# KVM-Explorer/AscendPathTracing

Hardware: AMD Instinct MI355X
Metric: Mray/s (ray segments per second) at 1920x1080, 8 bounces, 256 spp, demo scene (higher is better)
Workload: dtype f32; 1 GPU; C2: gen_spheres() 8-sphere scene, 1920x1080, S=64 (256 spp), depth 8, rays generated on device (counter RNG, seed 0), K-mode arithmetic, all segments traced (no retirement); segments_per_gpu=4246732800, parallelism=single GPU

## Files before the change

ascendpathtracing_amd/csrc/pt_trace2.h:

```cpp
#pragma once
#include <type_traits>

#include "pt_trace.h"

namespace {

template <bool PLANES, bool FIRST> constexpr int kPairSkip = !PLANES ? 0 : FIRST ? 0x8 : 0x80;
template <bool PLANES, bool FIRST> constexpr int kPairSkipLastB = 0;

struct PathPair {
    f2 ox, oy, oz, dx, dy, dz;
    f2 rx, ry, rz;
};

__device__ __forceinline__ PathState unpack_path(const PathPair &p, int which, uint64_t alive, bool first) {
    PathState s;
    if (which == 0) path_init(s, p.ox.x, p.oy.x, p.oz.x, p.dx.x, p.dy.x, p.dz.x);
    else path_init(s, p.ox.y, p.oy.y, p.oz.y, p.dx.y, p.dy.y, p.dz.y);
    if (first) return s;
    s.rxy = which == 0 ? f2{p.rx.x, p.ry.x} : f2{p.rx.y, p.ry.y};
    s.rz = which == 0 ? p.rz.x : p.rz.y;
    s.alive = select_const(alive, 1);
    return s;
}

template <int MODE, bool PLANES, bool FIRST>
__device__ __forceinline__ void bounce2_ns8_t(const Scene8 &sc, const Tab8 tab, const PathPair &s, PathPair &n,
                                              const TraceArgs &ta, const KeyConsts &kc, uint32_t ones_off,
                                              uint64_t &aliveA, uint64_t &aliveB, uint64_t &redoA, uint64_t &redoB) {
    float aminA = 1.0f, aminB = 1.0f;
    const Hit8 hA = intersect_ns8_v2<MODE, PLANES, kPairSkip<PLANES, FIRST>>(sc, s.ox.x, s.oy.x, s.oz.x, s.dx.x, s.dy.x, s.dz.x, ta, kc, aminA);
    const Hit8 hB = intersect_ns8_v2<MODE, PLANES, kPairSkip<PLANES, FIRST>>(sc, s.ox.y, s.oy.y, s.oz.y, s.dx.y, s.dy.y, s.dz.y, ta, kc, aminB);
    if (FIRST) {
        aliveA = ~hA.light;
        aliveB = ~hB.light;
    } else {
        aliveA &= ~hA.light;
        aliveB &= ~hB.light;
    }
    const char *geo = reinterpret_cast<const char *>(tab.geo);
    uint32_t cA, cB;
    asm("v_cndmask_b32_e64 %0, %1, %2, %3" : "=v"(cA) : "v"(ones_off), "v"(hA.addr), "s"(aliveA));
    asm("v_cndmask_b32_e64 %0, %1, %2, %3" : "=v"(cB) : "v"(ones_off), "v"(hB.addr), "s"(aliveB));
    const uint32_t gA = (uint32_t)(uintptr_t)geo + hA.addr, gB = (uint32_t)(uintptr_t)geo + hB.addr;
    const uint32_t aA = (uint32_t)(uintptr_t)geo + cA, aB = (uint32_t)(uintptr_t)geo + cB;
    float cxA, cyA, czA, cxB, cyB, czB, axA, ayA, azA, axB, ayB, azB;
    asm volatile("ds_read_b32 %0, %12\n ds_read_b32 %1, %12 offset:4\n ds_read_b32 %2, %12 offset:8\n"
                 "ds_read_b32 %3, %13\n ds_read_b32 %4, %13 offset:4\n ds_read_b32 %5, %13 offset:8\n"
                 "ds_read_b32 %6, %14 offset:128\n ds_read_b32 %7, %14 offset:132\n ds_read_b32 %8, %14 offset:136\n"
                 "ds_read_b32 %9, %15 offset:128\n ds_read_b32 %10, %15 offset:132\n ds_read_b32 %11, %15 offset:136\n"
                 "s_waitcnt lgkmcnt(0)"
                 : "=&v"(cxA), "=&v"(cyA), "=&v"(czA), "=&v"(cxB), "=&v"(cyB), "=&v"(czB), "=&v"(axA), "=&v"(ayA), "=&v"(azA),
                   "=&v"(axB), "=&v"(ayB), "=&v"(azB)
                 : "v"(gA), "v"(gB), "v"(aA), "v"(aB)
                 : "memory");
    const f2 cx = {cxA, cxB}, cy = {cyA, cyB}, cz = {czA, czB};
    const f2 ax = {axA, axB}, ay = {ayA, ayB}, az = {azA, azB};
    const f2 t = {hA.tmin, hB.tmin};
    const f2 hx = s.ox + s.dx * t, hy = s.oy + s.dy * t, hz = s.oz + s.dz * t;
    const f2 nx = hx - cx, ny = hy - cy, nz = hz - cz;
    f2 len2;
    if (MODE == kModeOracle) {
        const f2 p0 = nx * nx, p1 = ny * ny, p2 = nz * nz;
        len2 = f2{sum3_f64(p0.x, p1.x, p2.x), sum3_f64(p0.y, p1.y, p2.y)};
    } else {
        len2 = nx * nx + ny * ny;
        len2 = len2 + nz * nz;
    }
    const f2 r0 = {__builtin_amdgcn_rsqf(len2.x), __builtin_amdgcn_rsqf(len2.y)};
    aminA = minimum3_abs_after_trans(aminA, r0.x, nx.x);
    aminA = minimum3_abs(aminA, ny.x, nz.x);
    aminB = minimum3_abs_after_trans(aminB, r0.y, nx.y);
    aminB = minimum3_abs(aminB, ny.y, nz.y);
    const f2 L = sqrt_rsq_step(len2, r0);
    f2 ux, uy, uz, e1;
    div3_seeded_packed2(nx, ny, nz, L, r0, ux, uy, uz, e1);
    f2 dot;
    if (MODE == kModeOracle) {
        const f2 p0 = s.dx * ux, p1 = s.dy * uy, p2 = s.dz * uz;
        dot = f2{sum3_f64(p0.x, p1.x, p2.x), sum3_f64(p0.y, p1.y, p2.y)};
    } else {
        dot = s.dx * ux;
        dot = dot + s.dy * uy;
        dot = dot + s.dz * uz;
    }
    const f2 k2 = twice_canonical(dot);
    n.dx = s.dx - ux * k2; n.dy = s.dy - uy * k2; n.dz = s.dz - uz * k2;
    n.ox = hx; n.oy = hy; n.oz = hz;
    if (FIRST) { n.rx = ax; n.ry = ay; n.rz = az; }
    else { n.rx = ax * s.rx; n.ry = ay * s.ry; n.rz = az * s.rz; }
    redoA = __builtin_amdgcn_ballot_w64(!(aminA >= kFastMin)) | __builtin_amdgcn_ballot_w64(e1.x == kDiv3SeededStuck);
    redoB = __builtin_amdgcn_ballot_w64(!(aminB >= kFastMin)) | __builtin_amdgcn_ballot_w64(e1.y == kDiv3SeededStuck);
}
template <int MODE, bool PLANES>
__device__ __forceinline__ void bounce2_ns8(const Scene8 &sc, const Tab8 tab, const PathPair &s, PathPair &n,
                                            const TraceArgs &ta, const KeyConsts &kc, uint32_t ones_off,
                                            uint64_t &aliveA, uint64_t &aliveB, uint64_t &redoA, uint64_t &redoB) {
    bounce2_ns8_t<MODE, PLANES, false>(sc, tab, s, n, ta, kc, ones_off, aliveA, aliveB, redoA, redoB);
}
template <int MODE, bool PLANES>
__device__ __forceinline__ void bounce2_ns8_first(const Scene8 &sc, const Tab8 tab, const PathPair &s, PathPair &n,
                                                  const TraceArgs &ta, const KeyConsts &kc, uint32_t ones_off,
                                                  uint64_t &aliveA, uint64_t &aliveB, uint64_t &redoA, uint64_t &redoB) {
    bounce2_ns8_t<MODE, PLANES, true>(sc, tab, s, n, ta, kc, ones_off, aliveA, aliveB, redoA, redoB);
}

template <int MODE, bool PLANES, bool FIRST = false>
__device__ __forceinline__ void bounce2_ns8_last(const Scene8 &sc, const Tab8 tab, const PathPair &s, f2 &rx, f2 &ry, f2 &rz,
                                                 const TraceArgs &ta, const KeyConsts &kc, uint32_t ones_off,
                                                 uint64_t &aliveA, uint64_t &aliveB, uint64_t &redoA, uint64_t &redoB) {
    float aminA = 1.0f, aminB = 1.0f;
    const Hit8 hA = intersect_ns8_v2<MODE, PLANES, kPairSkip<PLANES, FIRST>>(sc, s.ox.x, s.oy.x, s.oz.x, s.dx.x, s.dy.x, s.dz.x, ta, kc, aminA);
    const Hit8 hB = intersect_ns8_v2<MODE, PLANES, kPairSkipLastB<PLANES, FIRST>>(sc, s.ox.y, s.oy.y, s.oz.y, s.dx.y, s.dy.y, s.dz.y, ta, kc, aminB);
    if (FIRST) {
        aliveA = ~hA.light;
        aliveB = ~hB.light;
    } else {
        aliveA &= ~hA.light;
        aliveB &= ~hB.light;
    }
    uint32_t cA, cB;
    asm("v_cndmask_b32_e64 %0, %1, %2, %3" : "=v"(cA) : "v"(ones_off), "v"(hA.addr), "s"(aliveA));
    asm("v_cndmask_b32_e64 %0, %1, %2, %3" : "=v"(cB) : "v"(ones_off), "v"(hB.addr), "s"(aliveB));
    const char *geo = reinterpret_cast<const char *>(tab.geo);
    const uint32_t aA = (uint32_t)(uintptr_t)geo + cA, aB = (uint32_t)(uintptr_t)geo + cB;
    float axA, ayA, azA, axB, ayB, azB;
    asm volatile("ds_read_b32 %0, %6 offset:128\n ds_read_b32 %1, %6 offset:132\n ds_read_b32 %2, %6 offset:136\n"
                 "ds_read_b32 %3, %7 offset:128\n ds_read_b32 %4, %7 offset:132\n ds_read_b32 %5, %7 offset:136\n"
                 "s_waitcnt lgkmcnt(0)"
                 : "=&v"(axA), "=&v"(ayA), "=&v"(azA), "=&v"(axB), "=&v"(ayB), "=&v"(azB)
                 : "v"(aA), "v"(aB)
                 : "memory");
    if (FIRST) { rx = f2{axA, axB}; ry = f2{ayA, ayB}; rz = f2{azA, azB}; }
    else { rx = f2{axA, axB} * s.rx; ry = f2{ayA, ayB} * s.ry; rz = f2{azA, azB} * s.rz; }
    redoA = __builtin_amdgcn_ballot_w64(!(aminA >= kFastMin));
    redoB = __builtin_amdgcn_ballot_w64(!(aminB >= kFastMin));
}

template <int MODE, bool PLANES>
__device__ __forceinline__ void trace2_ns8_t(const Scene8 &sc, const Tab8 tab, PathPair &s, const TraceArgs &ta) {
    const KeyConsts kc = make_key_consts(ta.eps);
    uint32_t ones_off = 8 * 16;
    asm volatile("" : "+v"(ones_off));
    uint64_t aliveA = __builtin_amdgcn_ballot_w64(true), aliveB = aliveA;
    const bool fast_ok = eps_allows_rootkey(ta.eps);
    auto redo_stands = [&](const PathPair &in, uint64_t redoA, uint64_t redoB, bool first) __attribute__((always_inline)) {
        if (first) return (redoA | redoB) != 0;
        const bool finA = select_const(aliveA, 1) == 0 || (in.rx.x == 0.0f && in.ry.x == 0.0f && in.rz.x == 0.0f);
        const bool finB = select_const(aliveB, 1) == 0 || (in.rx.y == 0.0f && in.ry.y == 0.0f && in.rz.y == 0.0f);
        return __builtin_amdgcn_ballot_w64((select_const(redoA, 1) != 0 && !finA) || (select_const(redoB, 1) != 0 && !finB)) != 0;
    };
    auto exact_pair = [&](const PathPair &in, PathState &na, PathState &nb, bool first) __attribute__((always_inline)) {
        PathState a = unpack_path(in, 0, aliveA, first), b = unpack_path(in, 1, aliveB, first);
        bounce_ns8_exact<MODE>(sc, tab, a, na, ta);
        bounce_ns8_exact<MODE>(sc, tab, b, nb, ta);
        if (ta.traced && (threadIdx.x & 63) == 0) atomicAdd(ta.traced + 3, 1ull);
    };
#ifdef APT_COUNT_PAIR_SKIP
    uint32_t count_bounce = 0;
    auto count_pairs = [&](const PathPair &in) __attribute__((always_inline)) {
        if (!ta.traced) return;
        const bool lane0 = (threadIdx.x & 63) == 0;
        for (int half = 0; half < 2; ++half) {
            const float ox = half ? in.ox.y : in.ox.x, oy = half ? in.oy.y : in.oy.x, oz = half ? in.oz.y : in.oz.x;
            const float dx = half ? in.dx.y : in.dx.x, dy = half ? in.dy.y : in.dy.x, dz = half ? in.dz.y : in.dz.x;
            HitPre2 hp[4];
            f2 c67 = {0.0f, 0.0f};
            if (PLANES) intersect_pre_planes<true>(sc, ox, oy, oz, dx, dy, dz, hp, &c67);
            for (int k = 0; k < 8; k += 2) {
                const HitPre2 h = PLANES ? hp[k / 2]
                                         : intersect_pre2(f2{sc.cx[k], sc.cx[k + 1]}, f2{sc.cy[k], sc.cy[k + 1]}, f2{sc.cz[k], sc.cz[k + 1]},
                                                          f2{sc.r2[k], sc.r2[k + 1]}, ox, oy, oz, dx, dy, dz);
                const uint32_t slot = 4u + (uint32_t)(half * 8 + (count_bounce < 7u ? count_bounce : 7u)) * 4u + (uint32_t)(k / 2);
                if (pair_misses_wave(h.disc) && lane0) atomicAdd(ta.traced + slot, 1ull);
                if (PLANES && k == 6) {
                    const uint32_t s67 = 72u + (uint32_t)(half * 8 + (count_bounce < 7u ? count_bounce : 7u)) * 4u;
                    const bool u6 = sphere_reachable_mask(h.disc.x, h.b.x, c67.x) == 0, u7 = sphere_reachable_mask(h.disc.y, h.b.y, c67.y) == 0;
                    const bool r6 = h.disc.x >= 0.0f && !(h.b.x < 0.0f && c67.x > 0.0f), r7 = h.disc.y >= 0.0f && !(h.b.y < 0.0f && c67.y > 0.0f);
                    const bool plain = __builtin_amdgcn_ballot_w64(r6 || r7) == 0;
                    if (u6 && lane0) atomicAdd(ta.traced + s67, 1ull);
                    if (u7 && lane0) atomicAdd(ta.traced + s67 + 1, 1ull);
                    if (u6 && u7 && lane0) atomicAdd(ta.traced + s67 + 2, 1ull);
                    if (plain && lane0) atomicAdd(ta.traced + s67 + 3, 1ull);
                }
            }
        }
        if (count_bounce == 0 && lane0) atomicAdd(ta.traced + 68, 1ull);
        ++count_bounce;
    };
#endif
    auto step = [&](const PathPair &in, PathPair &out, auto first_tag) __attribute__((always_inline)) {
        constexpr bool first = decltype(first_tag)::value;
#ifdef APT_COUNT_PAIR_SKIP
        count_pairs(in);
#endif
        uint64_t oa = aliveA, ob = aliveB;
        bool redo_any = !fast_ok;
        if (__builtin_expect(fast_ok, 1)) {
            uint64_t redoA, redoB;
            bounce2_ns8_t<MODE, PLANES, first>(sc, tab, in, out, ta, kc, ones_off, oa, ob, redoA, redoB);
            if (__builtin_expect((redoA | redoB) != 0, 0)) redo_any = redo_stands(in, redoA, redoB, first);
        }
        if (__builtin_expect(redo_any, 0)) {
            PathState na, nb;
            exact_pair(in, na, nb, first);
            out.ox = f2{na.oxy.x, nb.oxy.x}; out.oy = f2{na.oxy.y, nb.oxy.y}; out.oz = f2{na.oz, nb.oz};
            out.dx = f2{na.dxy.x, nb.dxy.x}; out.dy = f2{na.dxy.y, nb.dxy.y}; out.dz = f2{na.dz, nb.dz};
            out.rx = f2{na.rxy.x, nb.rxy.x}; out.ry = f2{na.rxy.y, nb.rxy.y}; out.rz = f2{na.rz, nb.rz};
            oa = __builtin_amdgcn_ballot_w64(na.alive != 0);
            ob = __builtin_amdgcn_ballot_w64(nb.alive != 0);
        }
        aliveA = oa; aliveB = ob;
    };
    auto last = [&](const PathPair &in, auto first_tag) __attribute__((always_inline)) {
        constexpr bool first = decltype(first_tag)::value;
#ifdef APT_COUNT_PAIR_SKIP
        count_pairs(in);
#endif
        uint64_t oa = aliveA, ob = aliveB;
        f2 rx, ry, rz;
        bool redo_any = !fast_ok;
        if (__builtin_expect(fast_ok, 1)) {
            uint64_t redoA, redoB;
            bounce2_ns8_last<MODE, PLANES, first>(sc, tab, in, rx, ry, rz, ta, kc, ones_off, oa, ob, redoA, redoB);
            if (__builtin_expect((redoA | redoB) != 0, 0)) redo_any = redo_stands(in, redoA, redoB, first);
        }
        if (__builtin_expect(redo_any, 0)) {
            PathState na, nb;
            exact_pair(in, na, nb, first);
            rx = f2{na.rxy.x, nb.rxy.x}; ry = f2{na.rxy.y, nb.rxy.y}; rz = f2{na.rz, nb.rz};
        }
        s.rx = rx; s.ry = ry; s.rz = rz;
    };
    using Yes = std::true_type;
    using No = std::false_type;
    if (ta.depth == 0) {
        const f2 one = {1.0f, 1.0f};
        s.rx = one; s.ry = one; s.rz = one;
        return;
    }
    if (ta.depth == 1) {
        last(s, Yes{});
        return;
    }
    const uint32_t full = ta.depth - 1;
    PathPair n;
    step(s, n, Yes{});
    uint32_t d = 1;
    for (; d + 2 <= full; d += 2) {
        step(n, s, No{});
        step(s, n, No{});
    }
    if (d < full) {
        step(n, s, No{});
        last(s, No{});
    } else {
        last(n, No{});
    }
}

template <int MODE>
__device__ __forceinline__ void trace2_ns8(const Scene8 &sc, const Tab8 tab, PathPair &s, const TraceArgs &ta, bool planes) {
    if (planes) trace2_ns8_t<MODE, true>(sc, tab, s, ta);
    else trace2_ns8_t<MODE, false>(sc, tab, s, ta);
}

}
```

profiles/pair_skip_count.py:

```python
#!/usr/bin/env python3
import argparse
import ctypes
import json
import os
import sys

sys.path.insert(0, os.path.dirname(os.path.dirname(os.path.abspath(__file__))))
import torch

import __graft_entry__

W, H, S, DEPTH = 1920, 1080, 64, 8
STAGE_CYCLES, TEST_CYCLES, PAIR_BOUNCE_CYCLES = 15 * 4.1 + 2 * 8.3, 2 * 4.1, 1250.0
ONE_STAGE_CYCLES = 11 * 4.1 + 1 * 8.3


def split_table(c, waves):
    T, F, O = TEST_CYCLES, STAGE_CYCLES, ONE_STAGE_CYCLES
    sites = []
    for h in (0, 1):
        for b in range(DEPTH):
            base = 72 + (h * 8 + b) * 4
            p6, p7, p67, plain = (c[base + j] / waves for j in range(4))
            pa = c[4 + (h * 8 + b) * 4 + 3] / waves
            cost = {"now": T + (1 - pa) * F,
                    "both": 2 * T + (p6 - p67) * O + (p7 - p67) * O + (1 - p6 - p7 + p67) * F,
                    "six_first": T + p6 * T + (p6 - p67) * O + (1 - p6) * F}
            best = min(cost, key=cost.get)
            last_b = h == 1 and b == DEPTH - 1
            valu_now = 15.0 if last_b else 2 + (1 - pa) * 15
            valu_built = valu_now if (b == 0 or last_b) else 4 + (p6 + p7 - 2 * p67) * 11 + (1 - p6 - p7 + p67) * 15
            cycles_now = F if last_b else cost["now"]
            cycles_built = cycles_now if (b == 0 or last_b) else cost["both"]
            sites.append({"path": "AB"[h], "bounce": b + 1, "U6": round(p6, 4), "U7": round(p7, 4), "U6_and_U7": round(p67, 4),
                          "U6_not_U7": round(p6 - p67, 4), "U7_not_U6": round(p7 - p67, 4), "U6_and_U7_unguarded": round(plain, 4),
                          "present_predicate": round(pa, 4), "cycles": {k: round(v, 2) for k, v in cost.items()}, "cheapest": best,
                          "saving_cycles": round(cost["now"] - cost[best], 2),
                          "built": "unchanged" if (b == 0 or last_b) else "both", "built_saving_cycles": round(cycles_now - cycles_built, 2),
                          "built_valu_instructions_saved": round(valu_now - valu_built, 3)})
    return sites


def main():
    here = os.path.dirname(os.path.abspath(__file__))
    ap = argparse.ArgumentParser()
    ap.add_argument("--out", default=os.path.join(here, "pair_skip_counts.json"))
    ap.add_argument("--general", action="store_true")
    ap.add_argument("--split-out", default=None)
    args = ap.parse_args()
    apt = __graft_entry__.build()
    from ascendpathtracing_amd import _lib, gen_data, render
    _lib.require_gpu()
    sph = torch.from_numpy(gen_data.gen_spheres()).cuda()
    if args.general:
        perm = sph.clone().view(-1)[:80].view(10, 8).clone()
        perm[:, [0, 6]] = perm[:, [6, 0]]
        sph[:80] = perm.reshape(-1)
    buf = torch.zeros(256, dtype=torch.int64, device="cuda")
    _lib.lib().apt_set_trace_counter(ctypes.c_void_p(buf.data_ptr()))
    render.render_frame(apt.make_params(W, H, S, depth=DEPTH), sph)
    torch.cuda.synchronize()
    _lib.lib().apt_set_trace_counter(None)
    c = buf.cpu().tolist()
    waves = c[68]
    assert waves > 0, "the library in APT_LIB_PATH is not the counting build"
    table = {}
    for pair in range(4):
        per = {h: [c[4 + (h * 8 + b) * 4 + pair] / waves for b in range(DEPTH)] for h in (0, 1)}
        p_bounce = [round((per[0][b] + per[1][b]) / 2, 4) for b in range(DEPTH)]
        p = sum(p_bounce) / DEPTH
        table[f"pair_{2 * pair}_{2 * pair + 1}"] = {
            "P_per_bounce": p_bounce, "P_path_A_per_bounce": [round(x, 4) for x in per[0]], "P_path_B_per_bounce": [round(x, 4) for x in per[1]],
            "P_mean": round(p, 4),
            "predicted_net_gain_of_a_pair_bounce": round(2 * (p * STAGE_CYCLES - TEST_CYCLES) / PAIR_BOUNCE_CYCLES, 5),
            "predicted_valu_per_segment": round(p * 15 - 2, 3)}
    out = {"what": "share P of the (wave, path half, bounce) triples of one C2 frame in which no lane can hit either sphere of the pair "
                   "(predicate (a): both discriminants negative or NaN in all 64 lanes)",
           "launch": "render_frame_kernel<0, 0, 8, false, true>", "frame": f"{W}x{H}, S={S}, depth {DEPTH}", "scene": "general (spheres 0 and 6 exchanged)" if args.general else "gen_spheres()",
           "device": torch.cuda.get_device_name(0), "wave_pair_traces": waves, "segments_traced": c[0], "exact_reruns": c[3], "pairs": table}
    with open(args.out, "w") as f:
        json.dump(out, f, indent=1)
        f.write("\n")
    print(json.dumps(out))
    if args.split_out:
        sites = split_table(c, waves)
        per_form = {k: round(sum(s["cycles"]["now"] - s["cycles"][k] for s in sites) / DEPTH, 2) for k in ("both", "six_first")}
        split = {"what": "pair (6,7) of one C2 frame: share of the waves in which every lane satisfies U6 / U7 (the sphere cannot be hit: "
                         "sphere_reachable_mask() is 0), per path half and bounce, and the cycles per path-bounce of each order of tests",
                 "launch": out["launch"], "frame": out["frame"], "scene": out["scene"], "device": out["device"], "wave_pair_traces": waves,
                 "price_model": f"VALU 4.1, transcendental 8.3 cycles: test {TEST_CYCLES:.1f}, full stage {STAGE_CYCLES:.1f}, "
                                f"one-sphere stage {ONE_STAGE_CYCLES:.1f}, pair-bounce {PAIR_BOUNCE_CYCLES:.0f}",
                 "sites": sites,
                 "saving_cycles_per_pair_bounce_one_form_everywhere": per_form,
                 "saving_cycles_per_pair_bounce_cheapest_per_site": round(sum(s["saving_cycles"] for s in sites) / DEPTH, 2),
                 "go_threshold_cycles": round(0.015 * PAIR_BOUNCE_CYCLES, 2),
                 "built_saving_cycles_per_pair_bounce": round(sum(s["built_saving_cycles"] for s in sites) / DEPTH, 2),
                 "built_predicted_valu_instructions_per_segment_saved": round(sum(s["built_valu_instructions_saved"] for s in sites) / (2 * DEPTH), 3)}
        with open(args.split_out, "w") as f:
            json.dump(split, f, indent=1)
            f.write("\n")
        print(json.dumps(split))


if __name__ == "__main__":
    main()
```

Baseline: 241,300 Mray/s.

## Intersect both paths of a pair jointly over shared plane-sphere coordinates

```diff
diff --git a/ascendpathtracing_amd/csrc/pt_trace2.h b/ascendpathtracing_amd/csrc/pt_trace2.h
--- a/ascendpathtracing_amd/csrc/pt_trace2.h
+++ b/ascendpathtracing_amd/csrc/pt_trace2.h
@@ -4,13 +4,13 @@
 #include "pt_trace.h"
 
 namespace {
-
-template <bool PLANES, bool FIRST> constexpr int kPairSkip = !PLANES ? 0 : FIRST ? 0x8 : 0x80;
-template <bool PLANES, bool FIRST> constexpr int kPairSkipLastB = 0;
 
 struct PathPair {
     f2 ox, oy, oz, dx, dy, dz;
     f2 rx, ry, rz;
+#ifdef APT_COUNT_PAIR_SKIP
+    uint32_t hitA, hitB;
+#endif
 };
 
 __device__ __forceinline__ PathState unpack_path(const PathPair &p, int which, uint64_t alive, bool first) {
@@ -24,13 +24,118 @@
     return s;
 }
 
+template <int MODE>
+struct ArgMin8 {
+    uint32_t best;
+    uint64_t b0 = 0, b1 = 0, b2 = 0, any = 0;
+    __device__ __forceinline__ void update64(uint64_t keys, int k) {
+        const uint32_t nb = min3_u32(best, (uint32_t)keys, (uint32_t)(keys >> 32));
+        const uint64_t better = __builtin_amdgcn_ballot_w64(nb != best);
+        best = nb;
+        b0 = (k & 1) ? (b0 | better) : (b0 & ~better);
+        b1 = (k & 2) ? (b1 | better) : (b1 & ~better);
+        b2 = (k & 4) ? (b2 | better) : (b2 & ~better);
+        if (MODE == kModeOracle) any |= better;
+    }
+    __device__ __forceinline__ Hit8 finish(const TraceArgs &ta, const KeyConsts &kc) {
+        const float tmin = bits_f32(best + kc.bias);
+        if (MODE == kModeOracle) { b0 |= ~any; b1 |= ~any; b2 |= ~any; }
+        uint32_t addr;
+        {
+            const uint32_t a0 = select_const(b0, 16), a1 = select_const(b1, 32), a2 = select_const(b2, 64);
+            asm("v_or3_b32 %0, %1, %2, %3" : "=v"(addr) : "v"(a0), "v"(a1), "v"(a2));
+        }
+        uint64_t light_mask = __builtin_amdgcn_ballot_w64(addr == (uint32_t)ta.light * 16u);
+        if (MODE == kModeOracle) light_mask &= any;
+        return Hit8{tmin, addr, light_mask};
+    }
+};
+
+template <int HALF>
+__device__ __forceinline__ f2 pair_half_minus(f2 cpair, f2 v) {
+    f2 r;
+    if (HALF == 0) asm("v_pk_add_f32 %0, %1, %2 op_sel:[0,0] op_sel_hi:[0,1] neg_lo:[0,1] neg_hi:[0,1]" : "=v"(r) : "s"(cpair), "v"(v));
+    else asm("v_pk_add_f32 %0, %1, %2 op_sel:[1,0] op_sel_hi:[1,1] neg_lo:[0,1] neg_hi:[0,1]" : "=v"(r) : "s"(cpair), "v"(v));
+    return r;
+}
+template <int HALF>
+__device__ __forceinline__ f2 minus_pair_half(f2 v, f2 cpair) {
+    f2 r;
+    if (HALF == 0) asm("v_pk_add_f32 %0, %1, %2 op_sel:[0,0] op_sel_hi:[1,0] neg_lo:[0,1] neg_hi:[0,1]" : "=v"(r) : "v"(v), "s"(cpair));
+    else asm("v_pk_add_f32 %0, %1, %2 op_sel:[0,1] op_sel_hi:[1,1] neg_lo:[0,1] neg_hi:[0,1]" : "=v"(r) : "v"(v), "s"(cpair));
+    return r;
+}
+
+constexpr int kAbSkip = 0xC0;
+
+template <int MODE, int SKIP>
+__device__ __forceinline__ void intersect2_ns8_planes(const Scene8 &sc, const PathPair &s, const TraceArgs &ta, const KeyConsts &kc,
+                                                      float &aminA, float &aminB, Hit8 &hA, Hit8 &hB) {
+    struct Term { f2 p, q; };
+    auto term = [](auto half, f2 cpair, f2 o, f2 d) __attribute__((always_inline)) {
+        const f2 t = pair_half_minus<decltype(half)::value>(cpair, o);
+        return Term{t * d, t * t};
+    };
+    struct Pre { f2 b, c, disc; };
+    auto pre = [](const Term &x, const Term &y, const Term &z, auto half, f2 r2pair) __attribute__((always_inline)) {
+        Pre h;
+        h.b = (x.p + y.p) + z.p;
+        h.c = minus_pair_half<decltype(half)::value>((x.q + y.q) + z.q, r2pair);
+        h.disc = h.b * h.b - h.c;
+        return h;
+    };
+    ArgMin8<MODE> A, B;
+    A.best = kc.init; B.best = kc.init;
+    auto stage = [&](const Pre &h, int k) __attribute__((always_inline)) {
+        const f2 q = sqrt_rn_rsq1_pair(h.disc);
+        A.update64(root_pair<0>(h.b, q) + kc.nbias2, k);
+        B.update64(root_pair<1>(h.b, q) + kc.nbias2, k);
+    };
+    auto walls = [&](const Pre &h0, const Pre &h1, int k) __attribute__((always_inline)) {
+        aminA = minimum3_abs(aminA, h0.disc.x, h1.disc.x);
+        aminB = minimum3_abs(aminB, h0.disc.y, h1.disc.y);
+        stage(h0, k);
+        stage(h1, k + 1);
+    };
+    auto tested = [&](const Pre &h, int k) __attribute__((always_inline)) {
+        if ((SKIP >> k) & 1) {
+            const float mA = __builtin_amdgcn_fmed3f(h.disc.x, h.b.x, -h.c.x), mB = __builtin_amdgcn_fmed3f(h.disc.y, h.b.y, -h.c.y);
+            uint32_t run = any_lane(__builtin_amdgcn_ballot_w64(__builtin_fmaxf(mA, mB) >= -kBehindGuard));
+            asm("" : "+s"(run));
+            if (run == 0u) return;
+        }
+        aminA = minimum3_abs(aminA, h.disc.x, h.disc.x);
+        aminB = minimum3_abs(aminB, h.disc.y, h.disc.y);
+        stage(h, k);
+    };
+    static_assert((SKIP & 0x3F) == 0, "the walls have no test: the room lies inside their spheres");
+    const f2 X1 = {sc.cx[0], sc.cx[1]}, X2 = {sc.cx[2], sc.cx[6]}, Y1 = {sc.cy[4], sc.cy[5]}, Y2 = {sc.cy[6], sc.cy[7]}, Y3 = {sc.cy[0], sc.cy[0]};
+    const f2 Z1 = {sc.cz[2], sc.cz[3]}, Z2 = {sc.cz[0], sc.cz[6]};
+    const f2 R0 = {sc.r2[0], sc.r2[1]}, R1 = {sc.r2[2], sc.r2[3]}, R2 = {sc.r2[4], sc.r2[5]}, R3 = {sc.r2[6], sc.r2[7]};
+    using Lo = std::integral_constant<int, 0>;
+    using Hi = std::integral_constant<int, 1>;
+    const Term x2 = term(Lo{}, X2, s.ox, s.dx), y0 = term(Lo{}, Y3, s.oy, s.dy), z0 = term(Lo{}, Z2, s.oz, s.dz);
+    walls(pre(term(Lo{}, X1, s.ox, s.dx), y0, z0, Lo{}, R0), pre(term(Hi{}, X1, s.ox, s.dx), y0, z0, Hi{}, R0), 0);
+    walls(pre(x2, y0, term(Lo{}, Z1, s.oz, s.dz), Lo{}, R1), pre(x2, y0, term(Hi{}, Z1, s.oz, s.dz), Hi{}, R1), 2);
+    walls(pre(x2, term(Lo{}, Y1, s.oy, s.dy), z0, Lo{}, R2), pre(x2, term(Hi{}, Y1, s.oy, s.dy), z0, Hi{}, R2), 4);
+    tested(pre(term(Hi{}, X2, s.ox, s.dx), term(Lo{}, Y2, s.oy, s.dy), term(Hi{}, Z2, s.oz, s.dz), Lo{}, R3), 6);
+    tested(pre(x2, term(Hi{}, Y2, s.oy, s.dy), z0, Hi{}, R3), 7);
+    hA = A.finish(ta, kc);
+    hB = B.finish(ta, kc);
+}
+
 template <int MODE, bool PLANES, bool FIRST>
 __device__ __forceinline__ void bounce2_ns8_t(const Scene8 &sc, const Tab8 tab, const PathPair &s, PathPair &n,
                                               const TraceArgs &ta, const KeyConsts &kc, uint32_t ones_off,
                                               uint64_t &aliveA, uint64_t &aliveB, uint64_t &redoA, uint64_t &redoB) {
     float aminA = 1.0f, aminB = 1.0f;
-    const Hit8 hA = intersect_ns8_v2<MODE, PLANES, kPairSkip<PLANES, FIRST>>(sc, s.ox.x, s.oy.x, s.oz.x, s.dx.x, s.dy.x, s.dz.x, ta, kc, aminA);
-    const Hit8 hB = intersect_ns8_v2<MODE, PLANES, kPairSkip<PLANES, FIRST>>(sc, s.ox.y, s.oy.y, s.oz.y, s.dx.y, s.dy.y, s.dz.y, ta, kc, aminB);
+    Hit8 hA, hB;
+    if (PLANES) {
+        intersect2_ns8_planes<MODE, kAbSkip>(sc, s, ta, kc, aminA, aminB, hA, hB);
+    } else {
+        hA = intersect_ns8_v2<MODE>(sc, s.ox.x, s.oy.x, s.oz.x, s.dx.x, s.dy.x, s.dz.x, ta, kc, aminA);
+        hB = intersect_ns8_v2<MODE>(sc, s.ox.y, s.oy.y, s.oz.y, s.dx.y, s.dy.y, s.dz.y, ta, kc, aminB);
+    }
     if (FIRST) {
         aliveA = ~hA.light;
         aliveB = ~hB.light;
@@ -91,6 +196,9 @@
     else { n.rx = ax * s.rx; n.ry = ay * s.ry; n.rz = az * s.rz; }
     redoA = __builtin_amdgcn_ballot_w64(!(aminA >= kFastMin)) | __builtin_amdgcn_ballot_w64(e1.x == kDiv3SeededStuck);
     redoB = __builtin_amdgcn_ballot_w64(!(aminB >= kFastMin)) | __builtin_amdgcn_ballot_w64(e1.y == kDiv3SeededStuck);
+#ifdef APT_COUNT_PAIR_SKIP
+    n.hitA = hA.addr; n.hitB = hB.addr;
+#endif
 }
 template <int MODE, bool PLANES>
 __device__ __forceinline__ void bounce2_ns8(const Scene8 &sc, const Tab8 tab, const PathPair &s, PathPair &n,
@@ -110,8 +218,13 @@
                                                  const TraceArgs &ta, const KeyConsts &kc, uint32_t ones_off,
                                                  uint64_t &aliveA, uint64_t &aliveB, uint64_t &redoA, uint64_t &redoB) {
     float aminA = 1.0f, aminB = 1.0f;
-    const Hit8 hA = intersect_ns8_v2<MODE, PLANES, kPairSkip<PLANES, FIRST>>(sc, s.ox.x, s.oy.x, s.oz.x, s.dx.x, s.dy.x, s.dz.x, ta, kc, aminA);
-    const Hit8 hB = intersect_ns8_v2<MODE, PLANES, kPairSkipLastB<PLANES, FIRST>>(sc, s.ox.y, s.oy.y, s.oz.y, s.dx.y, s.dy.y, s.dz.y, ta, kc, aminB);
+    Hit8 hA, hB;
+    if (PLANES) {
+        intersect2_ns8_planes<MODE, kAbSkip>(sc, s, ta, kc, aminA, aminB, hA, hB);
+    } else {
+        hA = intersect_ns8_v2<MODE>(sc, s.ox.x, s.oy.x, s.oz.x, s.dx.x, s.dy.x, s.dz.x, ta, kc, aminA);
+        hB = intersect_ns8_v2<MODE>(sc, s.ox.y, s.oy.y, s.oz.y, s.dx.y, s.dy.y, s.dz.y, ta, kc, aminB);
+    }
     if (FIRST) {
         aliveA = ~hA.light;
         aliveB = ~hB.light;
@@ -185,6 +298,49 @@
                 }
             }
         }
+        if (PLANES) {
+            const uint32_t bb = count_bounce < 7u ? count_bounce : 7u;
+            auto bcd = [&](int k, float ox, float oy, float oz, float dx, float dy, float dz, float &b, float &c, float &disc) {
+                const float x = sc.cx[k] - ox, y = sc.cy[k] - oy, z = sc.cz[k] - oz;
+                b = x * dx; b = b + y * dy; b = b + z * dz;
+                c = x * x; c = c + y * y; c = c + z * z; c = c - sc.r2[k];
+                disc = b * b; disc = disc - c;
+            };
+            bool strict[8], relaxed[8];
+            for (int k = 0; k < 8; ++k) {
+                float bA, cA, dA, bB, cB, dB;
+                bcd(k, in.ox.x, in.oy.x, in.oz.x, in.dx.x, in.dy.x, in.dz.x, bA, cA, dA);
+                bcd(k, in.ox.y, in.oy.y, in.oz.y, in.dx.y, in.dy.y, in.dz.y, bB, cB, dB);
+                const bool behindA = bA < -kBehindGuard, behindB = bB < -kBehindGuard;
+                const bool reach_s = __builtin_amdgcn_fmed3f(dA, bA, -cA) >= -kBehindGuard || __builtin_amdgcn_fmed3f(dB, bB, -cB) >= -kBehindGuard;
+                const bool reach_r = (dA >= 0.0f && !(behindA && cA >= 0.0f)) || (dB >= 0.0f && !(behindB && cB >= 0.0f));
+                const bool reach_ns = !(behindA && cA > kBehindGuard && behindB && cB > kBehindGuard);
+                const bool reach_nr = !(behindA && cA >= 0.0f && behindB && cB >= 0.0f);
+                strict[k] = __builtin_amdgcn_ballot_w64(reach_s) == 0;
+                relaxed[k] = __builtin_amdgcn_ballot_w64(reach_r) == 0;
+                if (strict[k] && lane0) atomicAdd(ta.traced + 136u + bb * 8u + (uint32_t)k, 1ull);
+                if (relaxed[k] && lane0) atomicAdd(ta.traced + 200u + bb * 8u + (uint32_t)k, 1ull);
+                if (__builtin_amdgcn_ballot_w64(reach_ns) == 0 && lane0) atomicAdd(ta.traced + 264u + bb * 8u + (uint32_t)k, 1ull);
+                if (__builtin_amdgcn_ballot_w64(reach_nr) == 0 && lane0) atomicAdd(ta.traced + 328u + bb * 8u + (uint32_t)k, 1ull);
+            }
+            if (count_bounce > 0) {
+                const uint32_t w = (uint32_t)__builtin_amdgcn_readfirstlane((int)in.hitA);
+                if (w < 6u * 16u && __builtin_amdgcn_ballot_w64(in.hitA != w || in.hitB != w) == 0) {
+                    const uint32_t k = w / 16u;
+                    bool s = false, r = false, opp = false;
+                    for (uint32_t j = 0; j < 6; ++j) {
+                        if (j == k) { s = strict[j]; r = relaxed[j]; }
+                        if (j == (k ^ 1u)) opp = strict[j];
+                    }
+                    if (lane0) {
+                        atomicAdd(ta.traced + 392u + bb * 4u, 1ull);
+                        if (s) atomicAdd(ta.traced + 393u + bb * 4u, 1ull);
+                        if (r) atomicAdd(ta.traced + 394u + bb * 4u, 1ull);
+                        if (opp) atomicAdd(ta.traced + 395u + bb * 4u, 1ull);
+                    }
+                }
+            }
+        }
         if (count_bounce == 0 && lane0) atomicAdd(ta.traced + 68, 1ull);
         ++count_bounce;
     };
@@ -209,6 +365,9 @@
             out.rx = f2{na.rxy.x, nb.rxy.x}; out.ry = f2{na.rxy.y, nb.rxy.y}; out.rz = f2{na.rz, nb.rz};
             oa = __builtin_amdgcn_ballot_w64(na.alive != 0);
             ob = __builtin_amdgcn_ballot_w64(nb.alive != 0);
+#ifdef APT_COUNT_PAIR_SKIP
+            out.hitA = ~0u; out.hitB = ~0u;
+#endif
         }
         aliveA = oa; aliveB = ob;
     };
@@ -261,8 +420,15 @@
 
 template <int MODE>
 __device__ __forceinline__ void trace2_ns8(const Scene8 &sc, const Tab8 tab, PathPair &s, const TraceArgs &ta, bool planes) {
-    if (planes) trace2_ns8_t<MODE, true>(sc, tab, s, ta);
-    else trace2_ns8_t<MODE, false>(sc, tab, s, ta);
-}
-
-}
+    if (planes) {
+        Scene8 p = sc;
+        p.cx[3] = p.cx[4] = p.cx[5] = p.cx[7] = sc.cx[2];
+        p.cy[1] = p.cy[2] = p.cy[3] = sc.cy[0];
+        p.cz[1] = p.cz[4] = p.cz[5] = p.cz[7] = sc.cz[0];
+        trace2_ns8_t<MODE, true>(p, tab, s, ta);
+    } else {
+        trace2_ns8_t<MODE, false>(sc, tab, s, ta);
+    }
+}
+
+}
diff --git a/profiles/pair_skip_count.py b/profiles/pair_skip_count.py
--- a/profiles/pair_skip_count.py
+++ b/profiles/pair_skip_count.py
@@ -41,12 +41,62 @@
     return sites
 
 
+AB_TEST_WALL, AB_TEST_DISC, AB_DISC_PAIR = 3 * 4.1, 4 * 4.1, 2 * 4.1
+AB_FEWER_PACKED = 3 * 4.1
+BOUNCE_SHARE_OF_FRAME = 0.86
+AB_GATE = 0.02
+
+
+def ab_table(c, waves):
+    F, O, T2 = STAGE_CYCLES, ONE_STAGE_CYCLES, TEST_CYCLES
+    sites = []
+    for b in range(DEPTH):
+        blk = lambda base: [c[base + b * 8 + k] / waves for k in range(8)]
+        strict, relaxed, nodisc, nodisc_relaxed = blk(136), blk(200), blk(264), blk(328)
+        walls, wall_gain, wall_gain_relaxed = [], 0.0, 0.0
+        for k in range(6):
+            g = nodisc[k] * (F + AB_DISC_PAIR) - AB_TEST_WALL
+            gr = nodisc_relaxed[k] * (F + AB_DISC_PAIR) - AB_TEST_WALL
+            wall_gain += max(g, 0.0)
+            wall_gain_relaxed += max(gr, 0.0)
+            walls.append({"sphere": k, "P": round(strict[k], 4), "P_relaxed": round(relaxed[k], 4), "P_no_disc": round(nodisc[k], 4),
+                          "P_no_disc_relaxed": round(nodisc_relaxed[k], 4), "gain_cycles": round(g, 2), "gain_cycles_relaxed": round(gr, 2),
+                          "test": "on" if g > 0 else "off"})
+        today67 = 0.0
+        for h in (0, 1):
+            pa = c[4 + (h * 8 + b) * 4 + 3] / waves
+            p6, p7, p67 = (c[72 + (h * 8 + b) * 4 + j] / waves for j in range(3))
+            if h == 1 and b == DEPTH - 1:
+                today67 += F
+            elif b == 0:
+                today67 += T2 + (1 - pa) * F
+            else:
+                today67 += 2 * T2 + (p6 - p67) * O + (p7 - p67) * O + (1 - p6 - p7 + p67) * F
+        new67, tests67 = 0.0, []
+        for k in (6, 7):
+            with_test = AB_TEST_DISC + (1 - strict[k]) * F - strict[k] * AB_DISC_PAIR
+            new67 += min(with_test, F)
+            tests67.append("on" if with_test < F else "off")
+        j = 392 + b * 4
+        left = {"waves_share": round(c[j] / waves, 4), "passes_strict": round(c[j + 1] / c[j], 4) if c[j] else None,
+                "passes_relaxed": round(c[j + 2] / c[j], 4) if c[j] else None, "opposite_passes_strict": round(c[j + 3] / c[j], 4) if c[j] else None}
+        total = wall_gain + (today67 - new67) + AB_FEWER_PACKED
+        sites.append({"bounce": b + 1, "walls": walls, "P_sphere_6": round(strict[6], 4), "P_sphere_7": round(strict[7], 4),
+                      "P_sphere_6_relaxed": round(relaxed[6], 4), "P_sphere_7_relaxed": round(relaxed[7], 4),
+                      "pair67_today_cycles": round(today67, 2), "pair67_new_cycles": round(new67, 2), "pair67_tests": tests67,
+                      "just_left_wall": left, "wall_gain_cycles": round(wall_gain, 2), "wall_gain_cycles_relaxed": round(wall_gain_relaxed, 2),
+                      "pair67_gain_cycles": round(today67 - new67, 2), "gain_cycles": round(total, 2),
+                      "gain_cycles_relaxed": round(total - wall_gain + wall_gain_relaxed, 2)})
+    return sites
+
+
 def main():
     here = os.path.dirname(os.path.abspath(__file__))
     ap = argparse.ArgumentParser()
     ap.add_argument("--out", default=os.path.join(here, "pair_skip_counts.json"))
     ap.add_argument("--general", action="store_true")
     ap.add_argument("--split-out", default=None)
+    ap.add_argument("--ab-out", default=None)
     args = ap.parse_args()
     apt = __graft_entry__.build()
     from ascendpathtracing_amd import _lib, gen_data, render
@@ -56,7 +106,7 @@
         perm = sph.clone().view(-1)[:80].view(10, 8).clone()
         perm[:, [0, 6]] = perm[:, [6, 0]]
         sph[:80] = perm.reshape(-1)
-    buf = torch.zeros(256, dtype=torch.int64, device="cuda")
+    buf = torch.zeros(512, dtype=torch.int64, device="cuda")
     _lib.lib().apt_set_trace_counter(ctypes.c_void_p(buf.data_ptr()))
     render.render_frame(apt.make_params(W, H, S, depth=DEPTH), sph)
     torch.cuda.synchronize()
@@ -100,6 +150,29 @@
             json.dump(split, f, indent=1)
             f.write("\n")
         print(json.dumps(split))
+    if args.ab_out:
+        assert not args.general, "the (A, B) counts are of the shared-planes form"
+        sites = ab_table(c, waves)
+        mean = sum(s["gain_cycles"] for s in sites) / DEPTH
+        mean_relaxed = sum(s["gain_cycles_relaxed"] for s in sites) / DEPTH
+        frame = mean / PAIR_BOUNCE_CYCLES * BOUNCE_SHARE_OF_FRAME
+        ab = {"what": "one C2 frame: per bounce and sphere, the share P of the waves in which no lane can hit the sphere in path A or in path B "
+                      "(disc < 0 or NaN, or b < -2^-60 and c > 2^-60; P_relaxed: c >= 0; P_no_disc: the second clause alone), the wall a whole wave "
+                      "has just left, and the price of a root stage packed over (A, B) per sphere with a joint test in front of it",
+              "launch": out["launch"], "frame": out["frame"], "scene": out["scene"], "device": out["device"], "wave_pair_traces": waves,
+              "price_model": f"VALU 4.1, transcendental 8.3 cycles: stage {STAGE_CYCLES:.1f}, wall test {AB_TEST_WALL:.1f}, test with discriminant "
+                             f"{AB_TEST_DISC:.1f}, the skipped sphere's two packed discriminant instructions {AB_DISC_PAIR:.1f}, three packed "
+                             f"instructions fewer per pair-bounce {AB_FEWER_PACKED:.1f}, pair-bounce {PAIR_BOUNCE_CYCLES:.0f}; the bounce blocks are "
+                             f"{BOUNCE_SHARE_OF_FRAME} of the frame's VALU instructions",
+              "sites": sites,
+              "gain_cycles_per_pair_bounce": round(mean, 2), "gain_cycles_per_pair_bounce_relaxed_guard": round(mean_relaxed, 2),
+              "gain_share_of_pair_bounce": round(mean / PAIR_BOUNCE_CYCLES, 4),
+              "priced_share_of_frame": round(frame, 4), "priced_share_of_frame_relaxed_guard": round(mean_relaxed / PAIR_BOUNCE_CYCLES * BOUNCE_SHARE_OF_FRAME, 4),
+              "gate_share_of_frame": AB_GATE, "gate": "passed" if frame >= AB_GATE else "not passed"}
+        with open(args.ab_out, "w") as f:
+            json.dump(ab, f, indent=1)
+            f.write("\n")
+        print(json.dumps(ab))
 
 
 if __name__ == "__main__":
```

After: 244,700 Mray/s, median of 6. +1.4%, better.
